# ssilverman16/particle_col_image_segmentation

Hardware: AMD Instinct MI355X
Metric: Mpixels/sec segmented (5-ch 1024x1024 TIFF), ROI mask IoU=1.0 (higher is better)
Workload: dtype f32 planes / u8 class maps / int32 labels / f64 ROI sums; 1 GPU; BASELINE config 2: batch of 64 frames 1024x1024x5 float32 per GPU, full kernel chain, inputs resident in HBM; frames_per_gpu=64, height=1024, width=1024, planes=5, parallelism=frames x1, launch=one hipGraph replay per step, 4 in flight, tie_fallback_frames_last_step=0, reference_nan_frames_rank0=0

## Files before the change

### particle_col_image_segmentation_amd/csrc/ccl.hip

```cpp
#include <type_traits>

#include "column_pass.h"
#include "tile_ops.h"

namespace pcseg {

constexpr int SCAN_PIX = 1024;

struct KeyEqU8 {
    const uint8_t *p;
    int W;
    int64_t n;
    __device__ __forceinline__ int operator()(int b, int r, int c) const { return p[b * n + rowoff(r, W) + c]; }
};
struct KeyNzU8 {
    const uint8_t *p;
    int W;
    int64_t n;
    __device__ __forceinline__ int operator()(int b, int r, int c) const { return p[b * n + rowoff(r, W) + c] != 0; }
};
struct KeyZeroU8 {
    const uint8_t *p;
    int W;
    int64_t n;
// ... 305 lines not shown
    int lead[RELABEL_Q], lead2[RELABEL_Q], root[RELABEL_Q], val[RELABEL_Q], val2[RELABEL_Q], head_lane[RELABEL_Q];
    bool third = false;
    const int lane = lane_id();
#pragma unroll
    for (int q = 0; q < RELABEL_Q; ++q) {
        const int pv[4] = {pq[q].x, pq[q].y, pq[q].z, pq[q].w};
        lead[q] = pv[0] >= 0 ? pv[0] : (pv[1] >= 0 ? pv[1] : (pv[2] >= 0 ? pv[2] : pv[3]));
        const int left = __shfl_up(lead[q], 1);
        const bool head = lane == 0 || lead[q] != left;
        const unsigned long long heads = __ballot(head);
        head_lane[q] = 63 - __clzll((long long)(heads & (~0ull >> (63 - lane))));
        root[q] = head ? lead[q] : -1;
        lead2[q] = -1;
#pragma unroll
        for (int j = 1; j < 4; ++j) {
            if (pv[j] < 0 || pv[j] == lead[q]) continue;
            if (lead2[q] < 0) lead2[q] = pv[j];
            else if (pv[j] != lead2[q]) third = true;
        }
    }
    relabel_chains(par, lab, blockoff, pred, b, n, nblk, chase, root, val, &bad);
    bool any2 = false;
#pragma unroll
    for (int q = 0; q < RELABEL_Q; ++q) {
        val[q] = __shfl(val[q], head_lane[q]);
        root[q] = lead2[q];
        any2 = any2 || lead2[q] >= 0;
    }
    if (__any(any2)) relabel_chains(par, lab, blockoff, pred, b, n, nblk, chase, root, val2, &bad);
#pragma unroll
    for (int q = 0; q < RELABEL_Q; ++q) {
        const int64_t i = i0 + (int64_t)q * SCAN_PIX;
        if (i >= n) continue;
        const int pv[4] = {pq[q].x, pq[q].y, pq[q].z, pq[q].w};
        int out[4];
#pragma unroll
        for (int j = 0; j < 4; ++j) {
            out[j] = 0;
            if (pv[j] < 0) continue;
            if (pv[j] == lead[q]) out[j] = val[q];
            else if (pv[j] == lead2[q]) out[j] = val2[q];
            else if (third) out[j] = relabel_decode(par, lab, blockoff, pred, b, n, nblk, pv[j], chase, &bad);
        }
        *reinterpret_cast<int4 *>(lab + i) = make_int4(out[0], out[1], out[2], out[3]);
    }
    if (bad && counts) counts[b] = -1;
}

struct CclWs {
    int *parent;
    int *blockcount;
    int nblk;
    int *corrupt;
};

static CclWs ccl_carve(Carver &cv, int B, int H, int W)
{
    int64_t n = (int64_t)H * W;
    CclWs ws;
    ws.nblk = (int)((n + SCAN_PIX - 1) / SCAN_PIX);
    ws.parent = cv.take<int>((size_t)B * n);
    ws.blockcount = cv.take<int>((size_t)B * ws.nblk);
    ws.corrupt = cv.take<int>((size_t)B);
    return ws;
}

struct DilateCclWs {
    unsigned *bits, *dil;
};
static DilateCclWs dilate_ccl_carve(Carver &cv, int B, int H, int W)
{
    const size_t words = (size_t)B * ((H + 31) / 32) * W;
    DilateCclWs ws;
    ws.bits = cv.take<unsigned>(words);
    ws.dil = cv.take<unsigned>(words);
    return ws;
}
static unsigned *dilate_ccl_runs_carve(Carver &cv, int B, int H, int W) { return cv.take<unsigned>((size_t)B * ((H + 31) / 32) * W); }

struct FillHolesWs : CclWs {
    uint8_t *flag;
};
static FillHolesWs fill_holes_carve(Carver &cv, int B, int H, int W)
{
    FillHolesWs ws;
    static_cast<CclWs &>(ws) = ccl_carve(cv, B, H, W);
    ws.flag = cv.take<uint8_t>((size_t)B * H * W);
    return ws;
}

struct LocmaxWs : CclWs {
    size_t nwords;
    unsigned long long *cbits;
    uint8_t *bad;
    int *nonconst;
};
static LocmaxWs locmax_carve(Carver &cv, int B, int H, int W)
{
    const size_t total = (size_t)B * H * W;
    LocmaxWs ws;
    static_cast<CclWs &>(ws) = ccl_carve(cv, B, H, W);
    ws.nwords = (total + 63) / 64;
    ws.cbits = cv.take<unsigned long long>(ws.nwords + 1);
    ws.bad = cv.take<uint8_t>(total);
    ws.nonconst = cv.take<int>(B);
    return ws;
}

struct OverlapWs : CclWs {
    int *area, *ov;
};
static OverlapWs overlap_carve(Carver &cv, int B, int H, int W)
{
    OverlapWs ws;
    static_cast<CclWs &>(ws) = ccl_carve(cv, B, H, W);
    ws.area = cv.take<int>((size_t)B * H * W);
    ws.ov = cv.take<int>((size_t)B * H * W);
    return ws;
}

template <typename KeyFn, bool CONN8>
static int ccl_roots(KeyFn keyfn, int *parent, int B, int H, int W, hipStream_t s, bool tile_pass_done = false, int *corrupt = nullptr)
{
    if (corrupt) PCSEG_CHECK_HIP(hipMemsetAsync(corrupt, 0, sizeof(int) * (size_t)B, s));
    dim3 tgrid((W + CCL_TW - 1) / CCL_TW, (H + CCL_TH - 1) / CCL_TH, B);
    if (!tile_pass_done) {
        PCSEG_LAUNCH((ccl_tile_kernel<KeyFn, CONN8>), tgrid, dim3(256), 0, s, keyfn, parent, H, W);
        PCSEG_CHECK_LAUNCH();
    }
    if (tgrid.x > 1 || tgrid.y > 1) {
        const int64_t border_px = (int64_t)((H - 1) / CCL_TH) * W + (int64_t)(CONN8 ? 2 : 1) * ((W - 1) / CCL_TW) * H;
        dim3 bgrid((unsigned)((border_px + 255) / 256), B);
        PCSEG_LAUNCH((ccl_border_kernel<KeyFn, CONN8>), bgrid, dim3(256), 0, s, keyfn, parent, H, W, corrupt);
        PCSEG_CHECK_LAUNCH();
    }
    return PCSEG_OK;
}

template <typename Pred>
static int ccl_compact(int *parent, int *blockcount, int nblk, int *labels, int *counts, Pred pred, bool flatten,
                       int B, int H, int W, hipStream_t s, int *corrupt = nullptr)
{
    int64_t n = (int64_t)H * W;
    dim3 grid(nblk, B);
    PCSEG_LAUNCH((ccl_flatten_count_kernel<Pred>), grid, dim3(256), 0, s, parent, labels, blockcount, pred, n, nblk, false, corrupt);
    PCSEG_CHECK_LAUNCH();
    PCSEG_LAUNCH(ccl_scan_blocks_kernel, dim3(B), dim3(256), 0, s, blockcount, counts, nblk, (const int *)corrupt);
    PCSEG_CHECK_LAUNCH();
    if ((n & 3) == 0 && (((uintptr_t)parent | (uintptr_t)labels) & 15) == 0) {
        const dim3 qgrid((unsigned)((n + SCAN_PIX * RELABEL_Q - 1) / (SCAN_PIX * RELABEL_Q)), B);
        PCSEG_LAUNCH((ccl_relabel_quads_kernel<Pred>), qgrid, dim3(256), 0, s, (const int *)parent, labels, (const int *)blockcount, pred, n,
                     nblk, flatten, counts);
    } else {
        PCSEG_LAUNCH((ccl_relabel_kernel<Pred>), grid, dim3(256), 0, s, (const int *)parent, labels, (const int *)blockcount, pred, n, nblk,
                     flatten, counts);
    }
    PCSEG_CHECK_LAUNCH();
    return PCSEG_OK;
}

template <typename KeyFn, bool CONN8>
static int ccl_full(KeyFn keyfn, int32_t *labels, int32_t *counts, int B, int H, int W, void *workspace,
                    size_t workspace_bytes, hipStream_t s)
{
    Carver cv(workspace, workspace_bytes);
    CclWs ws = ccl_carve(cv, B, H, W);
    if (!cv.ok()) {
        set_error("ccl: workspace too small (%zu < %zu)", workspace_bytes, cv.off);
        return PCSEG_ERR_WORKSPACE;
    }
    int rc = ccl_roots<KeyFn, CONN8>(keyfn, ws.parent, B, H, W, s, false, ws.corrupt);
    if (rc) return rc;
    return ccl_compact(ws.parent, ws.blockcount, ws.nblk, labels, counts, PredAll(), true, B, H, W, s, ws.corrupt);
}

int ccl_plan(void *workspace, size_t workspace_bytes, int B, int H, int W, CclPlan *plan, const char *who)
{
    Carver cv(workspace, workspace_bytes);
    CclWs ws = ccl_carve(cv, B, H, W);
    if (!cv.ok()) {
        set_error("%s: workspace too small (%zu < %zu)", who, workspace_bytes, cv.off);
        return PCSEG_ERR_WORKSPACE;
    }
    plan->parent = ws.parent;
    plan->blockcount = ws.blockcount;
    plan->nblk = ws.nblk;
    plan->corrupt = ws.corrupt;
    return PCSEG_OK;
}

int ccl_equal_u8_finish(const uint8_t *in, const CclPlan &plan, bool tile_pass_done, int *labels, int *counts, int B, int H, int W,
                        hipStream_t s)
{
    const KeyEqU8 keyfn{in, W, (int64_t)H * W};
    PCSEG_CHECK_HIP(hipMemsetAsync(plan.corrupt, 0, sizeof(int) * (size_t)B, s));
    dim3 tgrid((W + CCL_TW - 1) / CCL_TW, (H + CCL_TH - 1) / CCL_TH, B);
    if (!tile_pass_done) {
        PCSEG_LAUNCH((ccl_tile_kernel<KeyEqU8, true>), tgrid, dim3(256), 0, s, keyfn, plan.parent, H, W);
        PCSEG_CHECK_LAUNCH();
    }
    if (tgrid.x > 1 || tgrid.y > 1) {
        const int64_t border_px = (int64_t)((H - 1) / CCL_TH) * W + (int64_t)2 * ((W - 1) / CCL_TW) * H;
        dim3 bgrid((unsigned)((border_px + 255) / 256), B);
        PCSEG_LAUNCH((ccl_border_kernel<KeyEqU8, true>), bgrid, dim3(256), 0, s, keyfn, plan.parent, H, W, plan.corrupt);
        PCSEG_CHECK_LAUNCH();
    }
    return ccl_compact(plan.parent, plan.blockcount, plan.nblk, labels, counts, PredAll(), true, B, H, W, s, plan.corrupt);
}

__global__ void __launch_bounds__(256) roots_to_parent_kernel(const int *__restrict__ roots, int *__restrict__ parent, int64_t total)
{
    int64_t i = (int64_t)blockIdx.x * blockDim.x + threadIdx.x;
    if (i < total) parent[i] = roots[i] - 1;
}

struct MaskSet {
    unsigned long long bits[4];
    int n;
};
template <bool VEC>
__global__ void __launch_bounds__(256) set_bits_kernel(const uint8_t *__restrict__ in, MaskSet masks, unsigned *__restrict__ bits,
                                                        int H, int W, int nch, int B)
{
    constexpr int COLS = VEC ? 4 : 1;
    const int c = (blockIdx.x * 256 + threadIdx.x) * COLS;
    const int ch = blockIdx.y, b = blockIdx.z;
    if (c >= W) return;
    const uint8_t *src = in + (int64_t)b * H * W + c;
    unsigned w[4][COLS];
#pragma unroll
    for (int m = 0; m < 4; ++m)
#pragma unroll
        for (int j = 0; j < COLS; ++j) w[m][j] = 0;
#pragma unroll 1
    for (int j0 = 0; j0 < 32; j0 += 8) {
        unsigned v8[8];
#pragma unroll
        for (int j = 0; j < 8; ++j) {
            const uint8_t *at = src + rowoff(min(ch * 32 + j0 + j, H - 1), W);
            v8[j] = VEC ? *reinterpret_cast<const unsigned *>(at) : (unsigned)*at;
        }
#pragma unroll
        for (int j = 0; j < 8; ++j) {
#pragma unroll
            for (int q = 0; q < COLS; ++q) {
                const unsigned a = (v8[j] >> (8 * q)) & 255u;
                const unsigned long long sel = a < 64 ? (1ull << a) : 0ull;
#pragma unroll
                for (int m = 0; m < 4; ++m)
                    if (m < masks.n && (masks.bits[m] & sel)) w[m][q] |= 1u << (j0 + j);
            }
        }
    }
    {
        const int rows = min(32, H - ch * 32);
        const unsigned valid = col_valid(rows);
#pragma unroll
        for (int m = 0; m < 4; ++m)
#pragma unroll
            for (int q = 0; q < COLS; ++q) w[m][q] &= valid;
// ... 45 lines not shown
{
    const int c = blockIdx.x * 256 + threadIdx.x;
    const int ch = blockIdx.y, b = blockIdx.z;
    if (c >= W) return;
    const unsigned *base = in + (int64_t)b * nch * W;
    const int chu = max(ch - 1, 0), chd = min(ch + 1, nch - 1);
    const unsigned *rc = base + rowoff(ch, W), *ru = base + rowoff(chu, W), *rd = base + rowoff(chd, W);
    const int c1l = max(c - 1, 0), c2l = max(c - 2, 0), c1r = min(c + 1, W - 1), c2r = min(c + 2, W - 1);
    const unsigned w0 = rc[c], w1l = rc[c1l], w1r = rc[c1r], w2l = rc[c2l], w2r = rc[c2r];
    unsigned u0 = ru[c], u1l = ru[c1l], u1r = ru[c1r], d0 = rd[c], d1l = rd[c1l], d1r = rd[c1r];
    if (ch == 0) u0 = u1l = u1r = 0;
    if (ch + 1 >= nch) d0 = d1l = d1r = 0;
    const unsigned cur1 = w0 | w1l | w1r, prev1 = u0 | u1l | u1r, next1 = d0 | d1l | d1r;
    unsigned acc = cur1 | w2l | w2r;
    acc |= (cur1 << 1) | (prev1 >> 31) | (cur1 >> 1) | (next1 << 31);
    acc |= (w0 << 2) | (u0 >> 30) | (w0 >> 2) | (d0 << 30);
    const int rows = min(32, H - ch * 32);
    acc &= col_valid(rows);
    out[((int64_t)b * nch + ch) * W + c] = acc;
}

constexpr int BR_TW = 64, BR_CH = 4, BR_ROWS = 32 * BR_CH;

__device__ __forceinline__ int bitrun_start(unsigned word, int p)
{
    const unsigned below = ~word & ((1u << p) - 1u);
    return below ? 32 - __clz(below) : 0;
}

template <typename Link>
__device__ __forceinline__ void bitrun_left_links(unsigned w, unsigned wl, Link &&link)
{
    unsigned rest = wl ? w : 0u;
    while (rest) {
        const int a = __ffs(rest) - 1;
        const unsigned from_a = w >> a;
        const int len = from_a == 0xFFFFFFFFu ? 32 : __ffs(~from_a) - 1;
        const int e = a + len - 1;
        rest = e >= 31 ? 0u : rest & ~((2u << e) - 1u);
        const int lo = max(a - 1, 0), hi = min(e + 1, 31);
        unsigned m = wl & (hi == 31 ? 0xFFFFFFFFu : ((2u << hi) - 1u)) & ~((1u << lo) - 1u);
        while (m) {
            const int p = __ffs(m) - 1;
            const int st = bitrun_start(wl, p);
            const unsigned from_p = wl >> p;
            const int run_len = from_p == 0xFFFFFFFFu ? 32 : __ffs(~from_p) - 1;
            const int en = p + run_len - 1;
            m = en >= 31 ? 0u : m & ~((2u << en) - 1u);
            link(a, st);
        }
    }
}

__global__ void __launch_bounds__(256) bitrun_tile_kernel(const unsigned *__restrict__ bits, int *__restrict__ parent, int H, int W,
                                                           int nch)
{
    __shared__ unsigned sw[BR_CH][BR_TW];
    __shared__ int lpar[BR_ROWS * BR_TW];
    const int col = threadIdx.x & (BR_TW - 1), q = threadIdx.x >> 6;
    const int c0 = blockIdx.x * BR_TW, ch0 = blockIdx.y * BR_CH, b = blockIdx.z;
    const int c = c0 + col, ch = ch0 + q;
    const unsigned w = (c < W && ch < nch) ? bits[((int64_t)b * nch + ch) * W + c] : 0u;
    sw[q][col] = w;
    for (unsigned heads = w & ~(w << 1); heads; heads &= heads - 1) {
        const int node = (q * 32 + (__ffs(heads) - 1)) * BR_TW + col;
        lpar[node] = node;
    }
    __syncthreads();
    if (w) {
        if (col > 0)
            bitrun_left_links(w, sw[q][col - 1], [&](int a, int st) {
                unite_lds(lpar, (q * 32 + a) * BR_TW + col, (q * 32 + st) * BR_TW + col - 1);
            });
        if ((w & 1u) && q > 0) {
            const int node = (q * 32) * BR_TW + col;
            const unsigned wu = sw[q - 1][col];
            if (wu >> 31) {
                unite_lds(lpar, node, ((q - 1) * 32 + bitrun_start(wu, 31)) * BR_TW + col);
            } else {
                if (col > 0 && (sw[q - 1][col - 1] >> 31))
                    unite_lds(lpar, node, ((q - 1) * 32 + bitrun_start(sw[q - 1][col - 1], 31)) * BR_TW + col - 1);
                if (col + 1 < BR_TW && (sw[q - 1][col + 1] >> 31))
                    unite_lds(lpar, node, ((q - 1) * 32 + bitrun_start(sw[q - 1][col + 1], 31)) * BR_TW + col + 1);
            }
        }
    }
    __syncthreads();
    int *par = parent + (int64_t)b * H * W;
    for (unsigned heads = w & ~(w << 1); heads; heads &= heads - 1) {
        const int node = (q * 32 + (__ffs(heads) - 1)) * BR_TW + col;
        const int root = find_lds(lpar, node);
        par[(ch0 * 32 + node / BR_TW) * W + c0 + node % BR_TW] = (ch0 * 32 + root / BR_TW) * W + c0 + root % BR_TW;
    }
}

__global__ void __launch_bounds__(256) bitrun_border_kernel(const unsigned *__restrict__ bits, int *__restrict__ parent, int H, int W,
                                                             int nch)
{
    const int c = blockIdx.x * 256 + threadIdx.x;
    const int ch = blockIdx.y, b = blockIdx.z;
    if (c >= W) return;
    const int col = c & (BR_TW - 1);
    const bool tile_left = col == 0 && c > 0, tile_top = (ch % BR_CH) == 0 && ch > 0;
    const bool edge_col = col == 0 || col == BR_TW - 1;
    if (!tile_left && !tile_top && !(edge_col && ch > 0)) return;
    const unsigned *wb = bits + (int64_t)b * nch * W;
    const int cl = c > 0 ? c - 1 : c, cr = c + 1 < W ? c + 1 : c, chu = ch > 0 ? ch - 1 : ch;
    const unsigned w = wb[rowoff(ch, W) + c], wl = wb[rowoff(ch, W) + cl];
    const unsigned wu = wb[rowoff(chu, W) + c], wul = wb[rowoff(chu, W) + cl], wur = wb[rowoff(chu, W) + cr];
    if (w == 0) return;
    int *par = parent + (int64_t)b * H * W;
    const int row0 = ch * 32;
    if (tile_left)
        bitrun_left_links(w, wl, [&](int a, int st) { unite_glb(par, (row0 + a) * W + c, (row0 + st) * W + c - 1); });
    if ((w & 1u) && ch > 0) {
        const int node = row0 * W + c;
        if (wu >> 31) {
            if (tile_top) unite_glb(par, node, (row0 - 32 + bitrun_start(wu, 31)) * W + c);
        } else {
            if (c > 0 && (tile_top || col == 0) && (wul >> 31)) unite_glb(par, node, (row0 - 32 + bitrun_start(wul, 31)) * W + c - 1);
            if (c + 1 < W && (tile_top || col == BR_TW - 1) && (wur >> 31))
                unite_glb(par, node, (row0 - 32 + bitrun_start(wur, 31)) * W + c + 1);
        }
    }
}

__global__ void __launch_bounds__(256) border_flag_kernel(const int *__restrict__ parent, uint8_t *__restrict__ flag, int H, int W)
{
    int t = blockIdx.x * blockDim.x + threadIdx.x;
    int r, c;
    if (t < W) { r = 0; c = t; }
    else if (t < 2 * W) { r = H - 1; c = t - W; }
    else if (t < 2 * W + H) { r = t - 2 * W; c = 0; }
    else if (t < 2 * W + 2 * H) { r = t - 2 * W - H; c = W - 1; }
    else return;
    int64_t fbase = (int64_t)blockIdx.y * H * W;
    int p = parent[fbase + rowoff(r, W) + c];
    if (p >= 0) flag[fbase + p] = 1;
}

__global__ void __launch_bounds__(256) fill_holes_out_kernel(const uint8_t *__restrict__ mask, const int *__restrict__ parent,
                                                              const uint8_t *__restrict__ flag, uint8_t *__restrict__ out, int64_t n)
{
    int64_t i = (int64_t)blockIdx.x * blockDim.x + threadIdx.x;
    if (i >= n) return;
// ... 187 lines not shown
    unsigned long long w = cbits[g0 >> 6] >> sh;
    if (sh) w |= cbits[(g0 >> 6) + 1] << (64 - sh);
    if (n - i0 < 64) w &= (1ull << (n - i0)) - 1ull;
    return w;
}

static_assert(SCAN_PIX == 1024, "sixteen 64-bit words per count block");
template <typename Pred>
__global__ void __launch_bounds__(256) locmax_count_kernel(const int *__restrict__ parent, int *__restrict__ labels,
                                                            int *__restrict__ blockcount, const unsigned long long *__restrict__ cbits,
                                                            Pred pred, int64_t n, int nblk)
{
    const int b = blockIdx.y;
    const int *par = parent + (int64_t)b * n;
    const int64_t word = (int64_t)blockIdx.x * 256 + threadIdx.x;
    const int64_t i0 = word * 64;
    unsigned long long roots = 0;
    for (unsigned long long m = cand_word(cbits, b, i0, n); m; m &= m - 1) {
        const int j = __ffsll((long long)m) - 1;
        const int64_t i = i0 + j;
        if (par[i] == (int)i && pred((int64_t)b * n + i)) roots |= 1ull << j;
    }
    const int cnt = __popcll(roots);
    int inc = cnt;
    for (int off = 1; off < 16; off <<= 1) {
        const int t = __shfl_up(inc, off, 16);
        if ((threadIdx.x & 15) >= off) inc += t;
    }
    int rank = inc - cnt;
    for (unsigned long long m = roots; m; m &= m - 1) labels[(int64_t)b * n + i0 + (__ffsll((long long)m) - 1)] = -(++rank);
    if ((threadIdx.x & 15) == 15 && word / 16 < nblk) blockcount[b * nblk + (int)(word / 16)] = inc;
}

template <typename Pred>
__global__ void __launch_bounds__(256) locmax_relabel_kernel(const int *__restrict__ parent, int *labels, const int *__restrict__ blockoff,
                                                              const unsigned long long *__restrict__ cbits, Pred pred, int64_t n, int nblk)
{
    const int b = blockIdx.y;
    const int *par = parent + (int64_t)b * n;
    int *lab = labels + (int64_t)b * n;
    const int64_t i0 = ((int64_t)blockIdx.x * 256 + threadIdx.x) * 64;
    for (unsigned long long m = cand_word(cbits, b, i0, n); m; m &= m - 1) {
        const int64_t i = i0 + (__ffsll((long long)m) - 1);
        const int p = par[i];
        int v = 0;
        if (pred((int64_t)b * n + p)) {
            v = __hip_atomic_load(lab + p, __ATOMIC_RELAXED, __HIP_MEMORY_SCOPE_WORKGROUP);
            if (v < 0) v = blockoff[b * nblk + p / SCAN_PIX] - v;
        }
        lab[i] = v;
    }
}

__global__ void __launch_bounds__(256) overlap_count_kernel(const int *__restrict__ parent, const uint8_t *__restrict__ other,
                                                             int *__restrict__ area, int *__restrict__ ov, int64_t n)
{
    int64_t i = (int64_t)blockIdx.x * blockDim.x + threadIdx.x;
    if (i >= n) return;
    int64_t fbase = (int64_t)blockIdx.y * n;
    int p = parent[fbase + i];
    if (p < 0) return;
    atomicAdd(&area[fbase + p], 1);
    if (other[fbase + i] == 1) atomicAdd(&ov[fbase + p], 1);
}

__global__ void __launch_bounds__(256) overlap_out_kernel(const uint8_t *__restrict__ dapi, const int *__restrict__ parent,
                                                           const int *__restrict__ area, const int *__restrict__ ov,
                                                           double threshold, uint8_t *__restrict__ out, int64_t n)
{
    int64_t i = (int64_t)blockIdx.x * blockDim.x + threadIdx.x;
    if (i >= n) return;
    int64_t fbase = (int64_t)blockIdx.y * n;
    int p = parent[fbase + i];
    uint8_t v = dapi[fbase + i];
    if (p >= 0) {
        double frac = (double)ov[fbase + p] / (double)area[fbase + p];
        if (frac > threshold) v = 2;
    }
    out[fbase + i] = v;
}

}

using namespace pcseg;

extern "C" {

size_t pcseg_ccl_workspace_bytes(int B, int H, int W)
{
    if (!check_shape(B, H, W)) return 0;
    Carver cv(nullptr, 0);
    ccl_carve(cv, B, H, W);
    return cv.off;
}

int pcseg_ccl8_equal_u8(const uint8_t *in, int32_t *labels, int32_t *counts, int B, int H, int W, void *workspace,
                        size_t workspace_bytes, pcseg_stream_t stream)
{
    PCSEG_REQUIRE(in && labels && counts && workspace && check_shape(B, H, W), "bad arguments");
    return ccl_full<KeyEqU8, true>(KeyEqU8{in, W, (int64_t)H * W}, labels, counts, B, H, W, workspace, workspace_bytes, (hipStream_t)stream);
}

int pcseg_ccl8_bool(const uint8_t *in, int32_t *labels, int32_t *counts, int B, int H, int W, void *workspace,
                    size_t workspace_bytes, pcseg_stream_t stream)
{
    PCSEG_REQUIRE(in && labels && counts && workspace && check_shape(B, H, W), "bad arguments");
// ... 250 lines not shown
```

### particle_col_image_segmentation_amd/csrc/common.h

```cpp
#pragma once
#include <hip/hip_runtime.h>
#include <stdint.h>
#include <stdio.h>
#include <string.h>

#include "../../include/pcseg.h"

namespace pcseg {

constexpr int WAVE = 64;

void set_error(const char *fmt, ...);

#define PCSEG_CHECK_HIP(expr)                                                              \
    do {                                                                                   \
        hipError_t _e = (expr);                                                            \
        if (_e != hipSuccess) {                                                            \
            pcseg::set_error("%s failed: %s (%s:%d)", #expr, hipGetErrorString(_e), __FILE__, __LINE__); \
            return PCSEG_ERR_HIP;                                                          \
        }                                                                                  \
    } while (0)

#define PCSEG_CHECK_LAUNCH()                                                               \
    do {                                                                                   \
// ... 212 lines not shown
}

__device__ __forceinline__ int find_glb(int *par, int x, int *corrupt = nullptr)
{
    int p;
    while ((p = ld_agent(par + x)) != x) {
        if (!walk_ok(x, p)) { walk_corrupt(corrupt); return x; }
        int g = ld_agent(par + p);
        if (!walk_ok(p, g)) { walk_corrupt(corrupt); return p; }
        if (g != p) __hip_atomic_store(par + x, g, __ATOMIC_RELAXED, __HIP_MEMORY_SCOPE_AGENT);
        x = g;
    }
    return x;
}
__device__ __forceinline__ bool find2_glb(int *par, int &a, int &b, int *corrupt = nullptr)
{
    for (;;) {
        if (a == b) return true;
        const int pa = ld_agent(par + a), pb = ld_agent(par + b);
        if (pa == a && pb == b) return true;
        if (!walk_ok(a, pa) || !walk_ok(b, pb)) break;
        const int ga = ld_agent(par + pa), gb = ld_agent(par + pb);
        if (!walk_ok(pa, ga) || !walk_ok(pb, gb)) break;
        if (pa != a) {
            if (ga != pa) __hip_atomic_store(par + a, ga, __ATOMIC_RELAXED, __HIP_MEMORY_SCOPE_AGENT);
            a = ga;
        }
        if (pb != b) {
            if (gb != pb) __hip_atomic_store(par + b, gb, __ATOMIC_RELAXED, __HIP_MEMORY_SCOPE_AGENT);
            b = gb;
        }
    }
    walk_corrupt(corrupt);
    return false;
}
__device__ __forceinline__ void unite_glb(int *par, int a, int b, int *corrupt = nullptr)
{
    for (;;) {
        if (!find2_glb(par, a, b, corrupt)) return;
        if (a == b) return;
        if (a < b) { int t = a; a = b; b = t; }
        int old = atomicMin(par + a, b);
        if (old == a) return;
        if (!walk_ok(a, old)) { walk_corrupt(corrupt); return; }
        a = old;
    }
}

struct CclPlan {
    int *parent;
    int *blockcount;
    int nblk;
    int *corrupt;
};
int ccl_plan(void *workspace, size_t workspace_bytes, int B, int H, int W, CclPlan *plan, const char *who);
int ccl_equal_u8_finish(const uint8_t *in, const CclPlan &plan, bool tile_pass_done, int *labels, int *counts, int B, int H, int W,
                        hipStream_t s);

}
```

### particle_col_image_segmentation_amd/csrc/frontend.hip

```cpp
#include "common.h"
#include "tile_ops.h"

namespace pcseg {

template <int CT>
__device__ __forceinline__ unsigned classes4(const float *__restrict__ fr, int C, int64_t n, int64_t off)
{
    const int NC = CT > 0 ? CT : C;
    float4 v[CT > 0 ? CT : 1];
    if (CT > 0) {
#pragma unroll
        for (int k = 0; k < CT; ++k) v[k] = *reinterpret_cast<const float4 *>(fr + (int64_t)k * n + off);
    }
    float4 best = CT > 0 ? v[0] : *reinterpret_cast<const float4 *>(fr + off);
    unsigned a0 = 1, a1 = 1, a2 = 1, a3 = 1;
#pragma unroll
    for (int k = 1; k < NC; ++k) {
        const float4 x = CT > 0 ? v[CT > 0 ? k : 0] : *reinterpret_cast<const float4 *>(fr + (int64_t)k * n + off);
        if (x.x > best.x) { best.x = x.x; a0 = k + 1; }
        if (x.y > best.y) { best.y = x.y; a1 = k + 1; }
        if (x.z > best.z) { best.z = x.z; a2 = k + 1; }
        if (x.w > best.w) { best.w = x.w; a3 = k + 1; }
    }
    return a0 | (a1 << 8) | (a2 << 16) | (a3 << 24);
}

__device__ __forceinline__ unsigned class1(const float *__restrict__ fr, int C, int64_t n, int64_t off)
{
    float best = fr[off];
    unsigned arg = 1;
    for (int k = 1; k < C; ++k) {
        const float x = fr[(int64_t)k * n + off];
        if (x > best) { best = x; arg = k + 1; }
    }
    return arg;
}

template <int CT>
__global__ void __launch_bounds__(256, 1) classmap_median_ccl_kernel(const float *__restrict__ stack, int C, uint8_t *__restrict__ z,
                                                                   int *__restrict__ parent, int H, int W)
{
    __shared__ __attribute__((aligned(16))) uint32_t hot[MED_LH * MED_LW];
    __shared__ int key[CCL_TILE];
    static_assert(sizeof(uint32_t) * MED_LH * MED_LW >= sizeof(int) * CCL_TILE, "parents fit the histogram words");
    int *par = reinterpret_cast<int *>(hot);
    const TileIndex ti = xcd_tile_index();
    const int b = ti.z;
    const int r0 = ti.y * MED_TH, c0 = ti.x * MED_TW;
    const int64_t n = (int64_t)H * W;
    const float *fr = stack + (int64_t)b * C * n;
    const bool wide = c0 + MED_TW <= W && (W & 3) == 0 && ((uintptr_t)stack & 15) == 0;
    if (wide) {
        constexpr int QUADS = MED_LH * (MED_TW / 4), TRIPS = (QUADS + 255) / 256;
        unsigned cls4[TRIPS];
#pragma unroll
        for (int t = 0; t < TRIPS; ++t) {
            const int i = min((int)threadIdx.x + 256 * t, QUADS - 1);
            const int lr = i / (MED_TW / 4), q = i % (MED_TW / 4);
            int rr = r0 + lr - 2;
            rr = H >= 4 ? (rr < 0 ? -1 - rr : (rr >= H ? 2 * H - 1 - rr : rr)) : reflect_idx(rr, H);
            rr = min(max(rr, 0), H - 1);
            cls4[t] = classes4<CT>(fr, C, n, rowoff(rr, W) + c0 + 4 * q);
        }
#pragma unroll
        for (int t = 0; t < TRIPS; ++t) {
            const int i = (int)threadIdx.x + 256 * t;
            if (i < QUADS) {
                const int lr = i / (MED_TW / 4), q = i % (MED_TW / 4);
                const unsigned a = cls4[t];
                uint32_t *dst = hot + lr * MED_LW + 2 + 4 * q;
                dst[0] = 1u << (6 * (a & 255u) - 6);
                dst[1] = 1u << (6 * ((a >> 8) & 255u) - 6);
                dst[2] = 1u << (6 * ((a >> 16) & 255u) - 6);
                dst[3] = 1u << (6 * (a >> 24) - 6);
            }
        }
        for (int i = threadIdx.x; i < MED_LH * 4; i += 256) {
            const int lr = i >> 2, k = i & 3, lc = k < 2 ? k : MED_TW + k;
            int rr = r0 + lr - 2, cc = c0 + lc - 2;
            if (rr < 0 || rr >= H) rr = reflect_idx(rr, H);
            if (cc < 0 || cc >= W) cc = reflect_idx(cc, W);
            hot[lr * MED_LW + lc] = 1u << (6 * class1(fr, C, n, rowoff(rr, W) + cc) - 6);
        }
    } else {
        for (int i = threadIdx.x; i < MED_LH * (MED_TW + 4); i += 256) {
            const int lr = i / (MED_TW + 4), lc = i % (MED_TW + 4);
            int rr = r0 + lr - 2, cc = c0 + lc - 2;
            if (rr < 0 || rr >= H) rr = reflect_idx(rr, H);
            if (cc < 0 || cc >= W) cc = reflect_idx(cc, W);
            hot[lr * MED_LW + lc] = 1u << (6 * class1(fr, C, n, rowoff(rr, W) + cc) - 6);
        }
    }
    __syncthreads();
    uint8_t *dst = z + (int64_t)b * n;
    static_assert((MED_TW / 4) * (MED_TH / 2) == 256, "one pair of strips per thread");
    {
        const int s = threadIdx.x;
        const int lr = 2 * (s / (MED_TW / 4)), lc = (s % (MED_TW / 4)) * 4;
        const int c = c0 + lc;
        uint32_t med[2][4] = {{0, 0, 0, 0}, {0, 0, 0, 0}};
        if (r0 + lr < H && c < W) median5_hot6_strip2(hot, lr, lc, med[0], med[1]);
#pragma unroll
        for (int half = 0; half < 2; ++half) {
            const int r = r0 + lr + half;
#pragma unroll
            for (int j = 0; j < 4; ++j) key[(lr + half) * CCL_TW + lc + j] = (r < H && c + j < W) ? (int)med[half][j] : 0;
            if (r < H && c < W) {
                if (c + 3 < W && (W & 3) == 0) {
                    *reinterpret_cast<uint32_t *>(dst + rowoff(r, W) + c) =
                        med[half][0] | (med[half][1] << 8) | (med[half][2] << 16) | (med[half][3] << 24);
                } else {
                    for (int j = 0; j < 4 && c + j < W; ++j) dst[rowoff(r, W) + c + j] = (uint8_t)med[half][j];
                }
            }
        }
    }
    __syncthreads();
    ccl_tile_unions<true>(key, par);
    ccl_tile_store(key, par, parent, (int64_t)b * n, r0, c0, H, W);
}

static uint8_t *classmap_label_carve(Carver &cv, size_t ccl_bytes, int B, int H, int W)
{
    cv.take<uint8_t>(ccl_bytes);
    return cv.take<uint8_t>((size_t)B * H * W);
}

}

using namespace pcseg;

extern "C" {

size_t pcseg_classmap_label_workspace_bytes(int B, int H, int W)
{
    if (!check_shape(B, H, W)) return 0;
    Carver cv(nullptr, 0);
    classmap_label_carve(cv, pcseg_ccl_workspace_bytes(B, H, W), B, H, W);
    return cv.off;
}

int pcseg_classmap_label_f32(const float *stack, int C, uint8_t *denoised, int32_t *labels, int32_t *counts, int B, int H, int W,
                             void *workspace, size_t workspace_bytes, pcseg_stream_t stream)
{
    PCSEG_REQUIRE(stack && denoised && labels && counts && workspace && C >= 1 && C <= 255 && check_shape(B, H, W), "bad arguments");
    static_assert(MED_TW == CCL_TW && MED_TH == CCL_TH, "one tile shape for the median and the union-find");
    hipStream_t s = (hipStream_t)stream;
    const size_t ccl_bytes = pcseg_ccl_workspace_bytes(B, H, W);
    Carver cv(workspace, workspace_bytes);
    uint8_t *raw = classmap_label_carve(cv, ccl_bytes, B, H, W);
    PCSEG_REQUIRE(cv.ok(), "workspace too small");
    if (C > 5) {
        int rc = pcseg_argmax_planes_f32(stack, raw, B, C, H, W, stream);
        if (rc) return rc;
        rc = pcseg_median5_u8(raw, denoised, B, H, W, stream);
        if (rc) return rc;
        return pcseg_ccl8_equal_u8(denoised, labels, counts, B, H, W, workspace, ccl_bytes, stream);
    }
    CclPlan plan;
    int rc = ccl_plan(workspace, ccl_bytes, B, H, W, &plan, "classmap_label");
    if (rc) return rc;
    const dim3 grid((W + MED_TW - 1) / MED_TW, (H + MED_TH - 1) / MED_TH, B);
    if (C == 5)
        PCSEG_LAUNCH(classmap_median_ccl_kernel<5>, grid, dim3(256), 0, s, stack, C, denoised, plan.parent, H, W);
    else if (C == 4)
        PCSEG_LAUNCH(classmap_median_ccl_kernel<4>, grid, dim3(256), 0, s, stack, C, denoised, plan.parent, H, W);
    else if (C == 3)
        PCSEG_LAUNCH(classmap_median_ccl_kernel<3>, grid, dim3(256), 0, s, stack, C, denoised, plan.parent, H, W);
    else
        PCSEG_LAUNCH(classmap_median_ccl_kernel<0>, grid, dim3(256), 0, s, stack, C, denoised, plan.parent, H, W);
    PCSEG_CHECK_LAUNCH();
    return ccl_equal_u8_finish(denoised, plan, true, labels, counts, B, H, W, s);
}

}
```

### particle_col_image_segmentation_amd/csrc/tile_ops.h

```cpp
#pragma once
#include "common.h"

namespace pcseg {

constexpr int CCL_TW = 64, CCL_TH = 32, CCL_TILE = CCL_TW * CCL_TH;
static_assert(CCL_TH == 32 && CCL_TW == 64, "the tile pass assumes one 64-lane row per trip and one 32-row bit word per column");
constexpr int MED_TW = 64, MED_TH = 32, MED_LW = 72 , MED_LH = MED_TH + 4;

__device__ __forceinline__ int reflect_idx(int i, int n)
{
    int p = 2 * n;
    i %= p;
    if (i < 0) i += p;
    return i < n ? i : p - 1 - i;
}

__device__ __forceinline__ void median5_hot_strip(const uint32_t *hot, int lr, int lc, uint32_t med[4])
{
    uint32_t col[8] = {0, 0, 0, 0, 0, 0, 0, 0};
#pragma unroll
    for (int dr = 0; dr < 5; ++dr) {
        const uint4 *row = reinterpret_cast<const uint4 *>(hot + (lr + dr) * MED_LW + lc);
        const uint4 a = row[0], bq = row[1];
        col[0] += a.x; col[1] += a.y; col[2] += a.z; col[3] += a.w;
// ... 44 lines not shown
#pragma unroll
    for (int dr = 0; dr < 5; ++dr) {
        col[0] += a[dr].x; col[1] += a[dr].y; col[2] += a[dr].z; col[3] += a[dr].w;
        col[4] += bq[dr].x; col[5] += bq[dr].y; col[6] += bq[dr].z; col[7] += bq[dr].w;
    }
#pragma unroll
    for (int half = 0; half < 2; ++half) {
        if (half) {
            col[0] += a[5].x - a[0].x; col[1] += a[5].y - a[0].y; col[2] += a[5].z - a[0].z; col[3] += a[5].w - a[0].w;
            col[4] += bq[5].x - bq[0].x; col[5] += bq[5].y - bq[0].y; col[6] += bq[5].z - bq[0].z; col[7] += bq[5].w - bq[0].w;
        }
        uint32_t w = col[0] + col[1] + col[2] + col[3] + col[4];
#pragma unroll
        for (int j = 0; j < 4; ++j) {
            if (j > 0) w += col[j + 4] - col[j - 1];
            const uint32_t below = 0x2CB2CB2Cu - w * 0x01041041u;
            (half ? med1 : med0)[j] = 1u + __popc(below & 0x00820820u);
        }
    }
}

template <bool CONN8>
__device__ __forceinline__ void ccl_tile_unions(const int *key, int *par)
{
    for (int i = threadIdx.x; i < CCL_TILE; i += 256) {
        const int k = key[i], lc = i % CCL_TW;
        if (__ballot(k != 0) == 0) {
            par[i] = -1;
            continue;
        }
        const bool head = lc == 0 || key[i - 1] != k;
        const unsigned long long heads = __ballot(head);
        const unsigned long long upto = heads & (lc == 63 ? ~0ull : ((2ull << lc) - 1ull));
        const int start = 63 - __clzll((long long)upto);
        par[i] = k == 0 ? -1 : (i - lc + start);
    }
    __syncthreads();
    for (int i = threadIdx.x; i < CCL_TILE; i += 256) {
        int k = key[i], lc = i % CCL_TW;
        if (k == 0 || i < CCL_TW) continue;
        bool w = lc > 0 && key[i - 1] == k;
        bool n = key[i - CCL_TW] == k;
        bool nw = lc > 0 && key[i - CCL_TW - 1] == k;
        if (n && !(w && nw)) unite_lds_pair(par, i, i - CCL_TW);
        if (CONN8) {
            bool ne = lc < CCL_TW - 1 && key[i - CCL_TW + 1] == k;
            if (ne && !n) unite_lds_pair(par, i, i - CCL_TW + 1);
            if (nw && !n && !w) unite_lds_pair(par, i, i - CCL_TW - 1);
        }
    }
    __syncthreads();
}

__device__ __forceinline__ void ccl_tile_store(const int *key, int *par, int *__restrict__ parent, int64_t fbase, int r0, int c0,
                                               int H, int W)
{
    for (int i = threadIdx.x; i < CCL_TILE; i += 256) {
        int r = r0 + i / CCL_TW, c = c0 + i % CCL_TW;
        if (r >= H || c >= W) continue;
        int v = -1;
        if (key[i] != 0) {
            int root = find_lds(par, i);
            v = (r0 + root / CCL_TW) * W + c0 + root % CCL_TW;
        }
        parent[fbase + (int64_t)r * W + c] = v;
    }
}

}
```

Before: 16770 Mpixels/s.

## Record tile roots as bitmask to skip full flatten-count pass in classmap CCL

The fused median+CCL tile kernel now emits a per-pixel root bitmap via wave ballots, and a new count kernel walks only candidate root bits to assign provisional labels and block counts, replacing the full-image flatten_count pass. The bitrun tile kernel also switches to compact run-indexed LDS union-find nodes packed with position bits. The wide median load path absorbs the horizontal halo into the vectorized quad loads instead of a separate scalar loop. This adds a bitmap workspace and memset, and leans on border merges keeping the root candidates valid.

New measurement: 17050 Mpixels/s, median of 5. Within noise of the previous version (+1.6%).

```diff
diff --git a/particle_col_image_segmentation_amd/csrc/ccl.hip b/particle_col_image_segmentation_amd/csrc/ccl.hip
--- a/particle_col_image_segmentation_amd/csrc/ccl.hip
+++ b/particle_col_image_segmentation_amd/csrc/ccl.hip
@@ -381,6 +381,8 @@
     int *blockcount;
     int nblk;
     int *corrupt;
+    unsigned long long *rootbits;
+    size_t rootwords;
 };
 
 static CclWs ccl_carve(Carver &cv, int B, int H, int W)
@@ -391,6 +393,8 @@
     ws.parent = cv.take<int>((size_t)B * n);
     ws.blockcount = cv.take<int>((size_t)B * ws.nblk);
     ws.corrupt = cv.take<int>((size_t)B);
+    ws.rootwords = ((size_t)B * n + 63) / 64;
+    ws.rootbits = cv.take<unsigned long long>(ws.rootwords + 1);
     return ws;
 }
 
@@ -467,13 +471,11 @@
 }
 
 template <typename Pred>
-static int ccl_compact(int *parent, int *blockcount, int nblk, int *labels, int *counts, Pred pred, bool flatten,
-                       int B, int H, int W, hipStream_t s, int *corrupt = nullptr)
+static int ccl_relabel_counted(int *parent, int *blockcount, int nblk, int *labels, int *counts, Pred pred, bool flatten, int B, int H,
+                               int W, hipStream_t s, int *corrupt)
 {
     int64_t n = (int64_t)H * W;
     dim3 grid(nblk, B);
-    PCSEG_LAUNCH((ccl_flatten_count_kernel<Pred>), grid, dim3(256), 0, s, parent, labels, blockcount, pred, n, nblk, false, corrupt);
-    PCSEG_CHECK_LAUNCH();
     PCSEG_LAUNCH(ccl_scan_blocks_kernel, dim3(B), dim3(256), 0, s, blockcount, counts, nblk, (const int *)corrupt);
     PCSEG_CHECK_LAUNCH();
     if ((n & 3) == 0 && (((uintptr_t)parent | (uintptr_t)labels) & 15) == 0) {
@@ -488,6 +490,17 @@
     return PCSEG_OK;
 }
 
+template <typename Pred>
+static int ccl_compact(int *parent, int *blockcount, int nblk, int *labels, int *counts, Pred pred, bool flatten,
+                       int B, int H, int W, hipStream_t s, int *corrupt = nullptr)
+{
+    int64_t n = (int64_t)H * W;
+    PCSEG_LAUNCH((ccl_flatten_count_kernel<Pred>), dim3(nblk, B), dim3(256), 0, s, parent, labels, blockcount, pred, n, nblk, false,
+                 corrupt);
+    PCSEG_CHECK_LAUNCH();
+    return ccl_relabel_counted(parent, blockcount, nblk, labels, counts, pred, flatten, B, H, W, s, corrupt);
+}
+
 template <typename KeyFn, bool CONN8>
 static int ccl_full(KeyFn keyfn, int32_t *labels, int32_t *counts, int B, int H, int W, void *workspace,
                     size_t workspace_bytes, hipStream_t s)
@@ -515,26 +528,8 @@
     plan->blockcount = ws.blockcount;
     plan->nblk = ws.nblk;
     plan->corrupt = ws.corrupt;
+    plan->rootbits = ws.rootbits;
     return PCSEG_OK;
-}
-
-int ccl_equal_u8_finish(const uint8_t *in, const CclPlan &plan, bool tile_pass_done, int *labels, int *counts, int B, int H, int W,
-                        hipStream_t s)
-{
-    const KeyEqU8 keyfn{in, W, (int64_t)H * W};
-    PCSEG_CHECK_HIP(hipMemsetAsync(plan.corrupt, 0, sizeof(int) * (size_t)B, s));
-    dim3 tgrid((W + CCL_TW - 1) / CCL_TW, (H + CCL_TH - 1) / CCL_TH, B);
-    if (!tile_pass_done) {
-        PCSEG_LAUNCH((ccl_tile_kernel<KeyEqU8, true>), tgrid, dim3(256), 0, s, keyfn, plan.parent, H, W);
-        PCSEG_CHECK_LAUNCH();
-    }
-    if (tgrid.x > 1 || tgrid.y > 1) {
-        const int64_t border_px = (int64_t)((H - 1) / CCL_TH) * W + (int64_t)2 * ((W - 1) / CCL_TW) * H;
-        dim3 bgrid((unsigned)((border_px + 255) / 256), B);
-        PCSEG_LAUNCH((ccl_border_kernel<KeyEqU8, true>), bgrid, dim3(256), 0, s, keyfn, plan.parent, H, W, plan.corrupt);
-        PCSEG_CHECK_LAUNCH();
-    }
-    return ccl_compact(plan.parent, plan.blockcount, plan.nblk, labels, counts, PredAll(), true, B, H, W, s, plan.corrupt);
 }
 
 __global__ void __launch_bounds__(256) roots_to_parent_kernel(const int *__restrict__ roots, int *__restrict__ parent, int64_t total)
@@ -686,45 +681,85 @@
     }
 }
 
+constexpr int BR_NODES = 16 * 256, BR_NODE_BITS = 12;
+static_assert(BR_ROWS * BR_TW <= (1 << (31 - BR_NODE_BITS)) && BR_NODES == 1 << BR_NODE_BITS, "an entry packs position and node");
+
+__device__ __forceinline__ int bitrun_find(int *lpar, int x)
+{
+    for (;;) {
+        const int v = ld_lds(lpar + x);
+        if ((v & (BR_NODES - 1)) == x) return v;
+        x = v & (BR_NODES - 1);
+    }
+}
+__device__ __forceinline__ void bitrun_unite(int *lpar, int a, int b)
+{
+    for (;;) {
+        int va = bitrun_find(lpar, a), vb = bitrun_find(lpar, b);
+        if (va == vb) return;
+        if (va < vb) { const int t = va; va = vb; vb = t; }
+        const int old = atomicMin(&lpar[va & (BR_NODES - 1)], vb);
+        if (old == va) return;
+        a = old & (BR_NODES - 1);
+        b = vb & (BR_NODES - 1);
+    }
+}
+__device__ __forceinline__ int bitrun_node(unsigned word, int base, int top)
+{
+    const unsigned heads = word & ~(word << 1);
+    return base + __popc(heads & ((2u << top) - 1u)) - 1;
+}
+
 __global__ void __launch_bounds__(256) bitrun_tile_kernel(const unsigned *__restrict__ bits, int *__restrict__ parent, int H, int W,
                                                            int nch)
 {
     __shared__ unsigned sw[BR_CH][BR_TW];
-    __shared__ int lpar[BR_ROWS * BR_TW];
+    __shared__ int sbase[BR_CH][BR_TW];
+    __shared__ int lpar[BR_NODES];
+    __shared__ int wsum[4];
     const int col = threadIdx.x & (BR_TW - 1), q = threadIdx.x >> 6;
     const int c0 = blockIdx.x * BR_TW, ch0 = blockIdx.y * BR_CH, b = blockIdx.z;
     const int c = c0 + col, ch = ch0 + q;
     const unsigned w = (c < W && ch < nch) ? bits[((int64_t)b * nch + ch) * W + c] : 0u;
     sw[q][col] = w;
-    for (unsigned heads = w & ~(w << 1); heads; heads &= heads - 1) {
-        const int node = (q * 32 + (__ffs(heads) - 1)) * BR_TW + col;
-        lpar[node] = node;
+    int total;
+    const int base = block_exclusive_scan<256>((int)__popc(w & ~(w << 1)), &total, wsum);
+    sbase[q][col] = base;
+    {
+        int node = base;
+        for (unsigned heads = w & ~(w << 1); heads; heads &= heads - 1, ++node)
+            lpar[node] = (((q * 32 + (__ffs(heads) - 1)) * BR_TW + col) << BR_NODE_BITS) | node;
     }
     __syncthreads();
     if (w) {
-        if (col > 0)
-            bitrun_left_links(w, sw[q][col - 1], [&](int a, int st) {
-                unite_lds(lpar, (q * 32 + a) * BR_TW + col, (q * 32 + st) * BR_TW + col - 1);
-            });
+        if (col > 0) {
+            const unsigned wl = sw[q][col - 1];
+            const int bl = sbase[q][col - 1];
+            bitrun_left_links(w, wl, [&](int a, int st) { bitrun_unite(lpar, bitrun_node(w, base, a), bitrun_node(wl, bl, st)); });
+        }
         if ((w & 1u) && q > 0) {
-            const int node = (q * 32) * BR_TW + col;
             const unsigned wu = sw[q - 1][col];
             if (wu >> 31) {
-                unite_lds(lpar, node, ((q - 1) * 32 + bitrun_start(wu, 31)) * BR_TW + col);
+                bitrun_unite(lpar, base, bitrun_node(wu, sbase[q - 1][col], bitrun_start(wu, 31)));
             } else {
-                if (col > 0 && (sw[q - 1][col - 1] >> 31))
-                    unite_lds(lpar, node, ((q - 1) * 32 + bitrun_start(sw[q - 1][col - 1], 31)) * BR_TW + col - 1);
-                if (col + 1 < BR_TW && (sw[q - 1][col + 1] >> 31))
-                    unite_lds(lpar, node, ((q - 1) * 32 + bitrun_start(sw[q - 1][col + 1], 31)) * BR_TW + col + 1);
+                if (col > 0 && (sw[q - 1][col - 1] >> 31)) {
+                    const unsigned wul = sw[q - 1][col - 1];
+                    bitrun_unite(lpar, base, bitrun_node(wul, sbase[q - 1][col - 1], bitrun_start(wul, 31)));
+                }
+                if (col + 1 < BR_TW && (sw[q - 1][col + 1] >> 31)) {
+                    const unsigned wur = sw[q - 1][col + 1];
+                    bitrun_unite(lpar, base, bitrun_node(wur, sbase[q - 1][col + 1], bitrun_start(wur, 31)));
+                }
             }
         }
     }
     __syncthreads();
     int *par = parent + (int64_t)b * H * W;
-    for (unsigned heads = w & ~(w << 1); heads; heads &= heads - 1) {
-        const int node = (q * 32 + (__ffs(heads) - 1)) * BR_TW + col;
-        const int root = find_lds(lpar, node);
-        par[(ch0 * 32 + node / BR_TW) * W + c0 + node % BR_TW] = (ch0 * 32 + root / BR_TW) * W + c0 + root % BR_TW;
+    int node = base;
+    for (unsigned heads = w & ~(w << 1); heads; heads &= heads - 1, ++node) {
+        const int top = __ffs(heads) - 1;
+        const int root = bitrun_find(lpar, node) >> BR_NODE_BITS;
+        par[(ch0 * 32 + q * 32 + top) * W + c] = (ch0 * 32 + root / BR_TW) * W + c0 + root % BR_TW;
     }
 }
 
@@ -1018,6 +1053,64 @@
     }
 }
 
+__global__ void __launch_bounds__(256) ccl_rootbits_count_kernel(const int *__restrict__ parent, int *__restrict__ labels,
+                                                                  int *__restrict__ blockcount,
+                                                                  const unsigned long long *__restrict__ rootbits, int64_t n, int nblk,
+                                                                  int *__restrict__ corrupt)
+{
+    const int b = blockIdx.y;
+    const int *par = parent + (int64_t)b * n;
+    const int64_t word = (int64_t)blockIdx.x * 256 + threadIdx.x;
+    const int64_t i0 = word * 64;
+    unsigned long long roots = 0;
+    bool broken = false;
+    for (unsigned long long m = cand_word(rootbits, b, i0, n); m; m &= m - 1) {
+        const int j = __ffsll((long long)m) - 1;
+        const int i = (int)(i0 + j), p = par[i];
+        broken = broken || !walk_ok(i, p);
+        if (p == i) roots |= 1ull << j;
+    }
+    if (broken) walk_corrupt(corrupt + b);
+    const int cnt = __popcll(roots);
+    int inc = cnt;
+    for (int off = 1; off < 16; off <<= 1) {
+        const int t = __shfl_up(inc, off, 16);
+        if ((threadIdx.x & 15) >= off) inc += t;
+    }
+    int rank = inc - cnt;
+    for (unsigned long long m = roots; m; m &= m - 1) labels[(int64_t)b * n + i0 + (__ffsll((long long)m) - 1)] = -(++rank);
+    if ((threadIdx.x & 15) == 15 && word / 16 < nblk) blockcount[b * nblk + (int)(word / 16)] = inc;
+}
+
+int ccl_rootbits_begin(const CclPlan &plan, int B, int H, int W, hipStream_t s)
+{
+    size_t bytes = sizeof(int) * (size_t)B;
+    if (!ccl_rootbits_aligned(W)) {
+        const size_t words = ((size_t)B * H * W + 63) / 64 + 1;
+        bytes = (size_t)((char *)(plan.rootbits + words) - (char *)plan.corrupt);
+    }
+    PCSEG_CHECK_HIP(hipMemsetAsync(plan.corrupt, 0, bytes, s));
+    return PCSEG_OK;
+}
+
+int ccl_rootbits_finish(const uint8_t *in, const CclPlan &plan, int *labels, int *counts, int B, int H, int W, hipStream_t s)
+{
+    const int64_t n = (int64_t)H * W;
+    const KeyEqU8 keyfn{in, W, n};
+    dim3 tgrid((W + CCL_TW - 1) / CCL_TW, (H + CCL_TH - 1) / CCL_TH, B);
+    if (tgrid.x > 1 || tgrid.y > 1) {
+        const int64_t border_px = (int64_t)((H - 1) / CCL_TH) * W + (int64_t)2 * ((W - 1) / CCL_TW) * H;
+        dim3 bgrid((unsigned)((border_px + 255) / 256), B);
+        PCSEG_LAUNCH((ccl_border_kernel<KeyEqU8, true>), bgrid, dim3(256), 0, s, keyfn, plan.parent, H, W, plan.corrupt);
+        PCSEG_CHECK_LAUNCH();
+    }
+    const dim3 cgrid((unsigned)(((n + 63) / 64 + 255) / 256), B);
+    PCSEG_LAUNCH(ccl_rootbits_count_kernel, cgrid, dim3(256), 0, s, (const int *)plan.parent, labels, plan.blockcount,
+                 (const unsigned long long *)plan.rootbits, n, plan.nblk, plan.corrupt);
+    PCSEG_CHECK_LAUNCH();
+    return ccl_relabel_counted(plan.parent, plan.blockcount, plan.nblk, labels, counts, PredAll(), true, B, H, W, s, plan.corrupt);
+}
+
 __global__ void __launch_bounds__(256) overlap_count_kernel(const int *__restrict__ parent, const uint8_t *__restrict__ other,
                                                              int *__restrict__ area, int *__restrict__ ov, int64_t n)
 {
diff --git a/particle_col_image_segmentation_amd/csrc/common.h b/particle_col_image_segmentation_amd/csrc/common.h
--- a/particle_col_image_segmentation_amd/csrc/common.h
+++ b/particle_col_image_segmentation_amd/csrc/common.h
@@ -288,9 +288,11 @@
     int *blockcount;
     int nblk;
     int *corrupt;
-};
+    unsigned long long *rootbits;
+};
+__host__ __device__ inline bool ccl_rootbits_aligned(int W) { return (W & 63) == 0; }
 int ccl_plan(void *workspace, size_t workspace_bytes, int B, int H, int W, CclPlan *plan, const char *who);
-int ccl_equal_u8_finish(const uint8_t *in, const CclPlan &plan, bool tile_pass_done, int *labels, int *counts, int B, int H, int W,
-                        hipStream_t s);
-
-}
+int ccl_rootbits_begin(const CclPlan &plan, int B, int H, int W, hipStream_t s);
+int ccl_rootbits_finish(const uint8_t *in, const CclPlan &plan, int *labels, int *counts, int B, int H, int W, hipStream_t s);
+
+}
diff --git a/particle_col_image_segmentation_amd/csrc/frontend.hip b/particle_col_image_segmentation_amd/csrc/frontend.hip
--- a/particle_col_image_segmentation_amd/csrc/frontend.hip
+++ b/particle_col_image_segmentation_amd/csrc/frontend.hip
@@ -38,7 +38,8 @@
 
 template <int CT>
 __global__ void __launch_bounds__(256, 1) classmap_median_ccl_kernel(const float *__restrict__ stack, int C, uint8_t *__restrict__ z,
-                                                                   int *__restrict__ parent, int H, int W)
+                                                                   int *__restrict__ parent,
+                                                                   unsigned long long *__restrict__ rootbits, int H, int W)
 {
     __shared__ __attribute__((aligned(16))) uint32_t hot[MED_LH * MED_LW];
     __shared__ int key[CCL_TILE];
@@ -51,36 +52,39 @@
     const float *fr = stack + (int64_t)b * C * n;
     const bool wide = c0 + MED_TW <= W && (W & 3) == 0 && ((uintptr_t)stack & 15) == 0;
     if (wide) {
-        constexpr int QUADS = MED_LH * (MED_TW / 4), TRIPS = (QUADS + 255) / 256;
+        constexpr int RQ = MED_TW / 4 + 2, QUADS = MED_LH * RQ, TRIPS = (QUADS + 255) / 256;
+        const bool edge_l = c0 == 0, edge_r = c0 + MED_TW == W;
         unsigned cls4[TRIPS];
 #pragma unroll
         for (int t = 0; t < TRIPS; ++t) {
             const int i = min((int)threadIdx.x + 256 * t, QUADS - 1);
-            const int lr = i / (MED_TW / 4), q = i % (MED_TW / 4);
+            const int lr = i / RQ, q = i % RQ - 1;
             int rr = r0 + lr - 2;
             rr = H >= 4 ? (rr < 0 ? -1 - rr : (rr >= H ? 2 * H - 1 - rr : rr)) : reflect_idx(rr, H);
             rr = min(max(rr, 0), H - 1);
-            cls4[t] = classes4<CT>(fr, C, n, rowoff(rr, W) + c0 + 4 * q);
+            const int cq = min(max(c0 + 4 * q, 0), W - 4);
+            cls4[t] = classes4<CT>(fr, C, n, rowoff(rr, W) + cq);
         }
 #pragma unroll
         for (int t = 0; t < TRIPS; ++t) {
             const int i = (int)threadIdx.x + 256 * t;
             if (i < QUADS) {
-                const int lr = i / (MED_TW / 4), q = i % (MED_TW / 4);
+                const int lr = i / RQ, q = i % RQ - 1;
                 const unsigned a = cls4[t];
-                uint32_t *dst = hot + lr * MED_LW + 2 + 4 * q;
-                dst[0] = 1u << (6 * (a & 255u) - 6);
-                dst[1] = 1u << (6 * ((a >> 8) & 255u) - 6);
-                dst[2] = 1u << (6 * ((a >> 16) & 255u) - 6);
-                dst[3] = 1u << (6 * (a >> 24) - 6);
+                if (q < 0 || q == MED_TW / 4) {
+                    const unsigned lo = q < 0 ? (edge_l ? (a >> 8) & 255u : (a >> 16) & 255u) : (edge_r ? a >> 24 : a & 255u);
+                    const unsigned hi = q < 0 ? (edge_l ? a & 255u : a >> 24) : (edge_r ? (a >> 16) & 255u : (a >> 8) & 255u);
+                    uint32_t *dst = hot + lr * MED_LW + (q < 0 ? 0 : MED_TW + 2);
+                    dst[0] = 1u << (6 * lo - 6);
+                    dst[1] = 1u << (6 * hi - 6);
+                } else {
+                    uint32_t *dst = hot + lr * MED_LW + 2 + 4 * q;
+                    dst[0] = 1u << (6 * (a & 255u) - 6);
+                    dst[1] = 1u << (6 * ((a >> 8) & 255u) - 6);
+                    dst[2] = 1u << (6 * ((a >> 16) & 255u) - 6);
+                    dst[3] = 1u << (6 * (a >> 24) - 6);
+                }
             }
-        }
-        for (int i = threadIdx.x; i < MED_LH * 4; i += 256) {
-            const int lr = i >> 2, k = i & 3, lc = k < 2 ? k : MED_TW + k;
-            int rr = r0 + lr - 2, cc = c0 + lc - 2;
-            if (rr < 0 || rr >= H) rr = reflect_idx(rr, H);
-            if (cc < 0 || cc >= W) cc = reflect_idx(cc, W);
-            hot[lr * MED_LW + lc] = 1u << (6 * class1(fr, C, n, rowoff(rr, W) + cc) - 6);
         }
     } else {
         for (int i = threadIdx.x; i < MED_LH * (MED_TW + 4); i += 256) {
@@ -117,7 +121,7 @@
     }
     __syncthreads();
     ccl_tile_unions<true>(key, par);
-    ccl_tile_store(key, par, parent, (int64_t)b * n, r0, c0, H, W);
+    ccl_tile_store<true>(key, par, parent, (int64_t)b * n, r0, c0, H, W, rootbits);
 }
 
 static uint8_t *classmap_label_carve(Carver &cv, size_t ccl_bytes, int B, int H, int W)
@@ -160,17 +164,19 @@
     CclPlan plan;
     int rc = ccl_plan(workspace, ccl_bytes, B, H, W, &plan, "classmap_label");
     if (rc) return rc;
+    rc = ccl_rootbits_begin(plan, B, H, W, s);
+    if (rc) return rc;
     const dim3 grid((W + MED_TW - 1) / MED_TW, (H + MED_TH - 1) / MED_TH, B);
     if (C == 5)
-        PCSEG_LAUNCH(classmap_median_ccl_kernel<5>, grid, dim3(256), 0, s, stack, C, denoised, plan.parent, H, W);
+        PCSEG_LAUNCH(classmap_median_ccl_kernel<5>, grid, dim3(256), 0, s, stack, C, denoised, plan.parent, plan.rootbits, H, W);
     else if (C == 4)
-        PCSEG_LAUNCH(classmap_median_ccl_kernel<4>, grid, dim3(256), 0, s, stack, C, denoised, plan.parent, H, W);
+        PCSEG_LAUNCH(classmap_median_ccl_kernel<4>, grid, dim3(256), 0, s, stack, C, denoised, plan.parent, plan.rootbits, H, W);
     else if (C == 3)
-        PCSEG_LAUNCH(classmap_median_ccl_kernel<3>, grid, dim3(256), 0, s, stack, C, denoised, plan.parent, H, W);
+        PCSEG_LAUNCH(classmap_median_ccl_kernel<3>, grid, dim3(256), 0, s, stack, C, denoised, plan.parent, plan.rootbits, H, W);
     else
-        PCSEG_LAUNCH(classmap_median_ccl_kernel<0>, grid, dim3(256), 0, s, stack, C, denoised, plan.parent, H, W);
+        PCSEG_LAUNCH(classmap_median_ccl_kernel<0>, grid, dim3(256), 0, s, stack, C, denoised, plan.parent, plan.rootbits, H, W);
     PCSEG_CHECK_LAUNCH();
-    return ccl_equal_u8_finish(denoised, plan, true, labels, counts, B, H, W, s);
+    return ccl_rootbits_finish(denoised, plan, labels, counts, B, H, W, s);
 }
 
 }
diff --git a/particle_col_image_segmentation_amd/csrc/tile_ops.h b/particle_col_image_segmentation_amd/csrc/tile_ops.h
--- a/particle_col_image_segmentation_amd/csrc/tile_ops.h
+++ b/particle_col_image_segmentation_amd/csrc/tile_ops.h
@@ -120,18 +120,40 @@
     __syncthreads();
 }
 
+template <bool ROOTBITS = false>
 __device__ __forceinline__ void ccl_tile_store(const int *key, int *par, int *__restrict__ parent, int64_t fbase, int r0, int c0,
-                                               int H, int W)
+                                               int H, int W, unsigned long long *__restrict__ rootbits = nullptr)
 {
-    for (int i = threadIdx.x; i < CCL_TILE; i += 256) {
+    unsigned long long rowbits = 0;
+    int trip = 0;
+    for (int i = threadIdx.x; i < CCL_TILE; i += 256, ++trip) {
         int r = r0 + i / CCL_TW, c = c0 + i % CCL_TW;
-        if (r >= H || c >= W) continue;
+        const bool in = r < H && c < W;
         int v = -1;
-        if (key[i] != 0) {
+        bool is_root = false;
+        if (in && key[i] != 0) {
             int root = find_lds(par, i);
             v = (r0 + root / CCL_TW) * W + c0 + root % CCL_TW;
+            is_root = root == i;
         }
-        parent[fbase + (int64_t)r * W + c] = v;
+        if (in) parent[fbase + (int64_t)r * W + c] = v;
+        if (ROOTBITS) {
+            const unsigned long long ballot = __ballot(is_root);
+            if (lane_id() == trip) rowbits = ballot;
+        }
+    }
+    if (ROOTBITS) {
+        const int r = r0 + threadIdx.x / WAVE + (256 / WAVE) * lane_id();
+        if (lane_id() < CCL_TILE / 256 && r < H) {
+            const int64_t g = fbase + rowoff(r, W) + c0;
+            if (ccl_rootbits_aligned(W)) {
+                rootbits[g >> 6] = rowbits;
+            } else if (rowbits) {
+                const int sh = (int)(g & 63);
+                atomicOr(rootbits + (g >> 6), rowbits << sh);
+                if (sh) atomicOr(rootbits + (g >> 6) + 1, rowbits >> (64 - sh));
+            }
+        }
     }
 }
 
```
